# kenziyuliu/ChineseCheckersAgent

Hardware: NVIDIA B200
Metric: env_steps_per_sec (higher is better)
Workload: dtype u64

## Files before the change

chinesecheckersagent_b200/csrc/ccx_device.cuh:

```cuda
#pragma once
#include <cstdint>
#include <cuda_runtime.h>

typedef unsigned long long u64;
typedef unsigned int u32;

#define CCX_HD __host__ __device__ __forceinline__
#ifdef __CUDA_ARCH__
#define ccx_popc(x) __popc(x)
#define ccx_popcll(x) __popcll(x)
#define ccx_umulhi(a, b) __umulhi((a), (b))
#define ccx_clz(x) __clz(x)
#define ccx_clzll(x) __clzll((long long)(x))
#define ccx_ffs(x) __ffs(x)
#else
#define ccx_popc(x) __builtin_popcount(x)
#define ccx_popcll(x) __builtin_popcountll(x)
#define ccx_umulhi(a, b) ((u32)(((u64)(u32)(a) * (u64)(u32)(b)) >> 32))
#define ccx_clz(x) ((x) ? __builtin_clz(x) : 32)
#define ccx_clzll(x) ((x) ? __builtin_clzll(x) : 64)
#define ccx_ffs(x) __builtin_ffs(x)
#endif

#define CCX_VALID 0x007F7F7F7F7F7F7FULL
// ... 330 lines not shown

CCX_HD void apply_move(Game &g, int id, int from, int to)
{
    g.occ_me ^= (1ULL << from) | (1ULL << to);
    g.cells_me = (g.cells_me & ~(0xFFULL << (8 * id))) | ((u64)to << (8 * id));
    u64 meta = g.meta;
    u64 ply = ((meta >> 32) + 1) & 0xFFFF;
    g.meta = (meta & 0xFFFF000000000000ULL) ^ (1ULL << 48) | (ply << 32) | ((meta & 0xFFFF) << 16) |
             (u64)from | ((u64)to << 8);
    u64 t;
    t = g.occ_me; g.occ_me = g.occ_op; g.occ_op = t;
    t = g.cells_me; g.cells_me = g.cells_op; g.cells_op = t;
}

CCX_HD void push_hist(u64 &lo, u64 &hi, int to)
{
    hi = (hi << 8) | (lo >> 56);
    lo = (lo << 8) | (u64)to;
}

CCX_HD int level_of(int cell) { return (cell >> 3) - (cell & 7) + 6; }

CCX_HD int winner_of(const Game &g)
{
    bool p2 = (g.meta >> 48) & 1;
    return check_win(p2 ? g.occ_op : g.occ_me, p2 ? g.occ_me : g.occ_op);
}

CCX_HD void reset_start(Game &g)
{
    g.occ_me = CCX_START_OCC1; g.occ_op = CCX_START_OCC2;
    g.cells_me = CCX_START_CELLS1; g.cells_op = CCX_START_CELLS2;
    g.meta = CCX_START_META;
}

CCX_HD int pick_random(const Game &g, const u64 (&dest)[6], u32 nonempty, u32 r0, u32 r1, int &from, int &to)
{
    int j = (int)ccx_umulhi(r0, nonempty);
    int id = 0, rank = 0; u64 m = 0;
#pragma unroll
    for (int k = 0; k < 6; k++) {
        bool ne = dest[k] != 0;
        if (ne && rank == j) { id = k; m = dest[k]; }
        rank += ne;
    }
    to = select64(m, ccx_umulhi(r1, (u32)ccx_popcll(m)));
    from = (int)((g.cells_me >> (8 * id)) & 0xFF);
    return id;
}

struct TriTables {
    const uint8_t *sT; const u64 *sNB, *sCI, *sO, *sOT, *sOD;
    const u32 *sSel;
};

CCX_HD void tri_build(u64 cells_a, u64 cells_b, const u64 *__restrict__ sOT, const u64 *__restrict__ sOD, u64 &occT, u64 &occD)
{
    occT = 0; occD = 0;
#pragma unroll
    for (int k = 0; k < 6; k++) {
        int a = (int)((cells_a >> (8 * k)) & 0x3F), b = (int)((cells_b >> (8 * k)) & 0x3F);
        occT |= sOT[a] | sOT[b];
        occD |= sOD[a] | sOD[b];
    }
}

CCX_HD void movegen_tri(u64 occ_all, u64 occT_all, u64 occD_all, u64 cells, u64 (&dest)[6], const TriTables &T)
{
#pragma unroll
    for (int k = 0; k < 6; k++) dest[k] = 0;
    int id = 0, cell = (int)(cells & 0x3F);
    u64 o = T.sO[cell], occ = occ_all & ~o, occT = occT_all & ~T.sOT[cell], occD = occD_all & ~T.sOD[cell];
    u64 todo = o, reach = 0;
    for (;;) {
        int c = 63 - ccx_clzll(todo);
        todo ^= T.sO[c];
        u64 nw = expand_cell_tri(c, occ, occT, occD, T.sT, T.sCI) & ~(reach | o);
        reach |= nw;
        todo |= nw;
        if (todo == 0) {
            u64 d = (T.sNB[cell] & ~occ) | reach;
#pragma unroll
            for (int k = 0; k < 6; k++) if (id == k) dest[k] = d;
            if (++id == 6) break;
            cell = (int)((cells >> (8 * id)) & 0x3F);
            o = T.sO[cell]; occ = occ_all & ~o; occT = occT_all & ~T.sOT[cell]; occD = occD_all & ~T.sOD[cell];
            todo = o; reach = 0;
        }
    }
}

struct JumpFill {
    u64 o, occ, occT, occD, todo, reach;
};

CCX_HD JumpFill fill_start(int cell, u64 occ_all, u64 occT_all, u64 occD_all, const TriTables &T)
{
    JumpFill f;
    f.o = 1ULL << cell;
    f.occ = occ_all & ~f.o; f.occT = occT_all & ~T.sOT[cell]; f.occD = occD_all & ~T.sOD[cell];
    f.todo = f.o; f.reach = 0;
    return f;
}

CCX_HD void fill_step(JumpFill &f, const TriTables &T)
{
    const int c = 63 - ccx_clzll(f.todo);
    f.todo ^= 1ULL << c;
    const u64 nw = expand_cell_tri(c, f.occ, f.occT, f.occD, T.sT, T.sCI) & ~(f.reach | f.o);
    f.reach |= nw;
    f.todo |= nw;
}

CCX_HD u32 walk_movable(u64 occ_me, u64 occ_all, u64 cells_me)
{
    const u64 w = occ_me & neighbours(~occ_all & CCX_VALID);
    u32 b = 0;
#pragma unroll
    for (int k = 0; k < 6; k++) b |= (u32)((w >> ((cells_me >> (8 * k)) & 0x3F)) & 1) << k;
    return b;
}

CCX_HD int pick_first_start(const Game &g, u64 occT_all, u64 occD_all, u32 r0, const TriTables &T, int &from, JumpFill &f)
{
    const u64 occ_all = g.occ_me | g.occ_op;
    u32 movable = walk_movable(g.occ_me, occ_all, g.cells_me);
    u32 nowalk = ~movable & 0x3Fu;
    while (nowalk) {
        const int k = ccx_ffs(nowalk) - 1;
        nowalk &= nowalk - 1;
// ... 44 lines not shown
    k -= up ? c : 0u;
    const u32 c1 = ccx_popc(w & 0xFFu), c2 = ccx_popc(w & 0xFFFFu), c3 = ccx_popc(w & 0xFFFFFFu);
    const bool p1 = k >= c1, p2 = k >= c2, p3 = k >= c3;
    const u32 below = p2 ? (p3 ? c3 : c2) : (p1 ? c1 : 0u);
    const u32 sh = p2 ? (p3 ? 24u : 16u) : (p1 ? 8u : 0u);
    const u32 v = (w >> sh) & 0xFFu, r = k - below;
    const u32 pos = r < (u32)ccx_popc(v & 0x7Fu) ? sel7_rank(sSel, v & 0x7Fu, r) : 7u;
    return (int)((up ? 32u : 0u) + sh + pos);
}

CCX_HD u32 walk_movable_step(u64 occ_me, u64 occ_all, u64 cells_me)
{
    const u64 w = (occ_me & neighbours(~occ_all & CCX_VALID)) << 8;
    const u32 slo = (u32)cells_me + 0x05060708u, shi = (u32)(cells_me >> 32) + 0x0304u;
    u32 b = 0;
#pragma unroll
    for (u32 k = 0; k < 6; k++) b |= (u32)(w >> ccx_byte_of(slo, shi, 0x8880u | k)) & (1u << k);
    return b;
}

#define CCX_DBASE_LO 0x78503018u
#define CCX_DBASE_HI 0x305078A8u
struct CarryCell { u32 rsel, csel, dsel, lp8, sh; };
CCX_HD CarryCell carry_cell(int c)
{
    const int r = c >> 3, col = c & 7, k = col - r;
    const u32 x = (u32)k + 0x8894u;
    const u32 base8 = ccx_byte_of(CCX_DBASE_LO, CCX_DBASE_HI, 0x8894u - (u32)k);
    CarryCell q;
    q.rsel = 0x8880u | (u32)r;
    q.csel = 0x8880u | (u32)col;
    q.dsel = x & ((x - 1u) | 7u);
    q.lp8 = base8 + 8u * (u32)(r < col ? r : col);
    q.sh = (u32)(k > -8 * k ? k : -8 * k);
    return q;
}

CCX_HD u64 expand_cell_carry(int c, u64 occ, u64 occT, u64 occD, const uint8_t *__restrict__ T3)
{
    CarryCell q = carry_cell(c);
    const int r8 = c & 0x38;
    const u32 row7 = ccx_byte_of((u32)occ, (u32)(occ >> 32), q.rsel);
    u64 L = (u64)T3[CCX_JT3_ROW + row7 * 64 + c] << r8;
    const u32 col7 = ccx_byte_of((u32)occT, (u32)(occT >> 32), q.csel);
    L |= *reinterpret_cast<const u64 *>(T3 + CCX_JT3_COL + col7 * 64 + r8) << (c & 7);
    const u32 dia7 = ccx_byte_of((u32)occD, (u32)(occD >> 32), q.dsel);
#ifdef __CUDA_ARCH__
    asm("" : "+r"(q.lp8));
#endif
    L |= *reinterpret_cast<const u64 *>(T3 + CCX_JT3_DIA + dia7 * (CCX_JT3_NLP * 8) + q.lp8) << q.sh;
    return L;
}

CCX_HD void fill_step_carry(JumpFill &f, const uint8_t *__restrict__ T3)
{
    const int h = ccx_flo((u32)(f.todo >> 32)) | 32, l = ccx_flo((u32)f.todo);
    const int c = h > l ? h : l;
    f.todo ^= 1ULL << c;
    const u64 nw = expand_cell_carry(c, f.occ, f.occT, f.occD, T3) & ~(f.reach | f.o);
    f.reach |= nw;
    f.todo |= nw;
}

CCX_HD JumpFill carry_fill_start(int from, u64 occ_all, u64 occT_all, u64 occD_all, const TriTables &T)
{
    JumpFill f;
    f.o = 1ULL << from;
    f.occ = occ_all & ~f.o; f.occT = occT_all & ~T.sOT[from]; f.occD = occD_all & ~T.sOD[from];
    f.todo = expand_cell_carry(from, occ_all, occT_all, occD_all, T.sT);
    f.reach = (T.sNB[from] & ~occ_all) | f.todo;
    return f;
}

CCX_HD int carry_ply_start(const Game &g, u64 occT_all, u64 occD_all, u32 r0, const TriTables &T, int &from, JumpFill &f)
{
    const u64 occ_all = g.occ_me | g.occ_op;
    u32 movable = walk_movable_step(g.occ_me, occ_all, g.cells_me);
    u32 nowalk = ~movable & 0x3Fu;
    while (nowalk) {
        const int k = ccx_ffs(nowalk) - 1;
        nowalk &= nowalk - 1;
        if (expand_cell_carry((int)((g.cells_me >> (8 * k)) & 0x3F), occ_all, occT_all, occD_all, T.sT)) movable |= 1u << k;
    }
    if (!movable) return -1;
    const int id = (int)sel7_rank(T.sSel, movable, ccx_umulhi(r0, (u32)ccx_popc(movable)));
    from = (int)ccx_byte_of((u32)g.cells_me, (u32)(g.cells_me >> 32), 0x8880u | (u32)id);
    f = carry_fill_start(from, occ_all, occT_all, occD_all, T);
    return id;
}

CCX_HD int carry_ply_to(const JumpFill &f, u32 r1, const TriTables &T)
{
    return select64_step(f.reach, ccx_umulhi(r1, (u32)ccx_popcll(f.reach)), T.sSel);
}

CCX_HD u64 diag_mask(int l)
{
    const u64 D0 = 0x0040201008040201ULL;
    int k = 6 - l;
    if (k >= 0) return (D0 << k) & ((1ULL << (8 * (7 - k))) - 1ULL) & CCX_VALID;
    return (D0 << (8 * (-k))) & CCX_VALID;
}

CCX_HD int greedy_candidates(const Game &g, const u64 (&dest)[6], u64 (&cand)[6])
{
    bool p2 = (g.meta >> 48) & 1;
    int dist[6], start[6];
    int max_dist = -100;
#pragma unroll
    for (int k = 0; k < 6; k++) {
        u32 levels = 0;
#pragma unroll
        for (int l = 0; l < 13; l++) {
            const u64 dm = diag_mask(l);
            levels |= (dest[k] & dm) ? (1u << l) : 0u;
        }
        start[k] = level_of((int)((g.cells_me >> (8 * k)) & 0xFF));
        int best_end = p2 ? (31 - ccx_clz(levels)) : (ccx_ffs(levels) - 1);
        dist[k] = levels ? (p2 ? best_end - start[k] : start[k] - best_end) : -100;
        max_dist = dist[k] > max_dist ? dist[k] : max_dist;
    }
    int s_star = p2 ? 100 : -100;
#pragma unroll
    for (int k = 0; k < 6; k++)
        if (dist[k] == max_dist) s_star = p2 ? (start[k] < s_star ? start[k] : s_star) : (start[k] > s_star ? start[k] : s_star);
    int total = 0;
    if (max_dist == -100) {
#pragma unroll
        for (int k = 0; k < 6; k++) cand[k] = 0;
        return 0;
    }
    u64 end_mask = diag_mask(p2 ? s_star + max_dist : s_star - max_dist);
#pragma unroll
    for (int k = 0; k < 6; k++) {
        cand[k] = (dist[k] == max_dist && start[k] == s_star) ? (dest[k] & end_mask) : 0;
        total += ccx_popcll(cand[k]);
    }
    return total;
}

// ... 34 lines not shown
```

chinesecheckersagent_b200/csrc/ccx_env.cu:

```cuda
#include <cuda_bf16.h>
#include <new>
#include <cstdlib>
#include "ccx_device.cuh"
#include "ccx_internal.h"

#ifndef CCX_GREEDY_DEFAULT_VARIANT
#define CCX_GREEDY_DEFAULT_VARIANT 1
#endif
#define ENV_THREADS 64
#define ENC_THREADS 128


__device__ __forceinline__ Game load_game(const u64 *__restrict__ st, int64_t n, int64_t i)
{
    u64 occ1 = st[0 * n + i], occ2 = st[1 * n + i], c1 = st[2 * n + i], c2 = st[3 * n + i];
    Game g;
    g.meta = st[4 * n + i];
    bool p2 = (g.meta >> 48) & 1;
    g.occ_me = p2 ? occ2 : occ1; g.occ_op = p2 ? occ1 : occ2;
    g.cells_me = p2 ? c2 : c1;   g.cells_op = p2 ? c1 : c2;
    return g;
}

__device__ __forceinline__ void store_game(u64 *__restrict__ st, int64_t n, int64_t i, const Game &g)
// ... 71 lines not shown
    if (i >= n) return;
    Game g = load_game(st, n, i);
    int f = from[i], t = to[i];
    int id = 0;
#pragma unroll
    for (int k = 5; k >= 0; k--) if (((g.cells_me >> (8 * k)) & 0xFF) == (u64)f) id = k;
    apply_move(g, id, f, t);
    store_game(st, n, i, g);
    u64 lo = st[5 * n + i], hi = st[6 * n + i];
    push_hist(lo, hi, t);
    st[5 * n + i] = lo; st[6 * n + i] = hi;
    winner[i] = (uint8_t)winner_of(g);
}

__global__ void __launch_bounds__(ENV_THREADS)
k_info(const u64 *__restrict__ st, int64_t n, int16_t *__restrict__ out)
{
    int64_t i = (int64_t)blockIdx.x * blockDim.x + threadIdx.x;
    if (i >= n) return;
    u64 occ1 = st[0 * n + i], occ2 = st[1 * n + i], c1 = st[2 * n + i], c2 = st[3 * n + i];
    int d1 = 70, d2 = -14;
#pragma unroll
    for (int k = 0; k < 6; k++) {
        d1 -= level_of((int)((c1 >> (8 * k)) & 0xFF)) + 1;
        d2 += level_of((int)((c2 >> (8 * k)) & 0xFF)) + 1;
    }
    out[i * 5 + 0] = (int16_t)check_win(occ1, occ2);
    out[i * 5 + 1] = (int16_t)__popcll(occ1 & CCX_TARGET_P1);
    out[i * 5 + 2] = (int16_t)__popcll(occ2 & CCX_TARGET_P2);
    out[i * 5 + 3] = (int16_t)d1;
    out[i * 5 + 4] = (int16_t)d2;
}


#define CCX_TRI_SMEM_BYTES (CCX_JT3_BYTES + 5 * 64 * 8)
template <int TPB, bool SEL = false>
__device__ __forceinline__ TriTables tri_tables_load(uint8_t *sAll, const uint8_t *__restrict__ jt3)
{
    u64 *sNB = reinterpret_cast<u64 *>(sAll + CCX_JT3_BYTES), *sCI = sNB + 64, *sO = sNB + 128, *sOT = sNB + 192, *sOD = sNB + 256;
    u32 *sSel = SEL ? reinterpret_cast<u32 *>(sAll + CCX_TRI_SMEM_BYTES) : nullptr;
    for (int q = threadIdx.x; q < CCX_JT3_BYTES / 16; q += TPB) reinterpret_cast<uint4 *>(sAll)[q] = reinterpret_cast<const uint4 *>(jt3)[q];
    for (int q = threadIdx.x; q < 64; q += TPB) {
        const bool on = (CCX_VALID >> q) & 1;
        sNB[q] = on ? (neighbours(1ULL << q) & CCX_VALID) : 0ULL;
        sCI[q] = on ? tri_cell_info(q) : 0ULL;
        sO[q] = 1ULL << q;
        sOT[q] = on ? 1ULL << tri_tbit(q) : 0ULL;
        sOD[q] = on ? 1ULL << tri_dbit(q) : 0ULL;
    }
    if (SEL)
        for (int q = threadIdx.x; q < 128; q += TPB) sSel[q] = sel7_entry((u32)q);
    __syncthreads();
    TriTables t = {sAll, sNB, sCI, sO, sOT, sOD, sSel};
    return t;
}

template <bool TRACE, int TPB, int MINB>
__global__ void __launch_bounds__(TPB, MINB, 1)
k_step_random_pick(u64 *__restrict__ st, int64_t n, int64_t gid0, u32 k0, u32 k1, u32 step0, int plies,
                   u64 *__restrict__ wins, u64 *__restrict__ trace, int64_t trace_games, const uint8_t *__restrict__ jt3)
{
    __shared__ __align__(16) uint8_t sAll[CCX_JT3_BYTES + 5 * 64 * 8];
    const TriTables T = tri_tables_load<TPB>(sAll, jt3);
    const int64_t i = (int64_t)blockIdx.x * TPB + threadIdx.x;
    if (i >= n) return;
    Game g = load_game(st, n, i);
    const u64 gid = (u64)(gid0 + i);
    u32 w1 = 0, w2 = 0;
    u64 occT_all, occD_all;
    tri_build(g.cells_me, g.cells_op, T.sOT, T.sOD, occT_all, occD_all);
    for (int t = 0; t < plies; t++) {
        u64 *row = nullptr;
        if (TRACE && i < trace_games) {
            row = trace + ((int64_t)t * trace_games + i) * CCX_TRACE_WORDS;
            u64 dest[6];
            movegen_tri(g.occ_me | g.occ_op, occT_all, occD_all, g.cells_me, dest, T);
            bool p2 = (g.meta >> 48) & 1;
            row[0] = p2 ? g.occ_op : g.occ_me; row[1] = p2 ? g.occ_me : g.occ_op;
            row[2] = p2 ? g.cells_op : g.cells_me; row[3] = p2 ? g.cells_me : g.cells_op;
            row[4] = g.meta & 0x00FFFFFFFFFFFFFFULL;
#pragma unroll
            for (int q = 0; q < 6; q++) row[5 + q] = dest[q];
            row[11] = 0xFFULL | (0xFFULL << 8) | (0xFFULL << 24);
        }
        Philox4 rnd = philox4x32_10(k0, k1, step0 + (u32)t, 0u, (u32)gid, (u32)(gid >> 32));
        int from, to;
        const int pid = pick_random_first(g, occT_all, occD_all, rnd.x, rnd.y, T, from, to);
        if (pid < 0) continue;
        apply_move(g, pid, from, to);
        occT_all ^= T.sOT[from] | T.sOT[to];
        occD_all ^= T.sOD[from] | T.sOD[to];
        const int win = winner_of(g);
        if (TRACE && row) row[11] = (u64)from | ((u64)to << 8) | ((u64)win << 16) | ((u64)pid << 24);
        if (win) { w1 += win == 1; w2 += win == 2; reset_start(g); tri_build(g.cells_me, g.cells_op, T.sOT, T.sOD, occT_all, occD_all); }
    }
    store_game(st, n, i, g);
    if (w1) atomicAdd(&wins[0], (u64)w1);
    if (w2) atomicAdd(&wins[1], (u64)w2);
}

template <bool TRACE, int TPB, int MINB, int K>
__global__ void __launch_bounds__(TPB, MINB, 1)
k_step_random_carry(u64 *__restrict__ st, int64_t n, int64_t gid0, u32 k0, u32 k1, u32 step0, int plies,
                    u64 *__restrict__ wins, u64 *__restrict__ trace, int64_t trace_games, const uint8_t *__restrict__ jt3)
{
    __shared__ __align__(16) uint8_t sAll[CCX_TRI_SMEM_BYTES + CCX_SEL7_BYTES];
    const TriTables T = tri_tables_load<TPB, true>(sAll, jt3);
    const int64_t i = (int64_t)blockIdx.x * TPB + threadIdx.x;
    if (i >= n) return;
    Game g = load_game(st, n, i);
    const u64 gid = (u64)(gid0 + i);
    u32 w1 = 0, w2 = 0;
    JumpFill f = {0, 0, 0, 0, 0, 0};
    tri_build(g.cells_me, g.cells_op, T.sOT, T.sOD, f.occT, f.occD);
    int t = 0, id = -1, from = 0;
    Philox4 rnd = philox4x32_10(k0, k1, step0, 0u, (u32)gid, (u32)(gid >> 32));
    u32 r1 = 0;
    for (;;) {
        if (!f.todo) {
            u64 occT_all = f.occT, occD_all = f.occD;
            if (id >= 0) {
                rnd = philox4x32_10(k0, k1, step0 + (u32)t + 1u, 0u, (u32)gid, (u32)(gid >> 32));
                const int to = carry_ply_to(f, r1, T);
                apply_move(g, id, from, to);
                occT_all |= T.sOT[to];
                occD_all |= T.sOD[to];
#ifdef __CUDA_ARCH__
                asm volatile("" ::"r"(rnd.x), "r"(rnd.y));
#endif
                const int win = winner_of(g);
                if (TRACE && i < trace_games)
                    trace[((int64_t)t * trace_games + i) * CCX_TRACE_WORDS + 11] = (u64)from | ((u64)to << 8) | ((u64)win << 16) | ((u64)id << 24);
                if (win) { w1 += win == 1; w2 += win == 2; reset_start(g); tri_build(g.cells_me, g.cells_op, T.sOT, T.sOD, occT_all, occD_all); }
                t++;
                id = -1;
            }
            for (; t < plies; t++) {
                if (TRACE && i < trace_games) {
                    u64 *row = trace + ((int64_t)t * trace_games + i) * CCX_TRACE_WORDS;
                    u64 dest[6];
                    movegen_tri(g.occ_me | g.occ_op, occT_all, occD_all, g.cells_me, dest, T);
                    bool p2 = (g.meta >> 48) & 1;
                    row[0] = p2 ? g.occ_op : g.occ_me; row[1] = p2 ? g.occ_me : g.occ_op;
                    row[2] = p2 ? g.cells_op : g.cells_me; row[3] = p2 ? g.cells_me : g.cells_op;
                    row[4] = g.meta & 0x00FFFFFFFFFFFFFFULL;
#pragma unroll
                    for (int q = 0; q < 6; q++) row[5 + q] = dest[q];
                    row[11] = 0xFFULL | (0xFFULL << 8) | (0xFFULL << 24);
                }
                r1 = rnd.y;
                id = carry_ply_start(g, occT_all, occD_all, rnd.x, T, from, f);
                if (id >= 0) break;
                rnd = philox4x32_10(k0, k1, step0 + (u32)t + 1u, 0u, (u32)gid, (u32)(gid >> 32));
            }
            if (id < 0) break;
        }
#pragma unroll
        for (int k = 0; k < K; k++) { if (!f.todo) break; fill_step_carry(f, T.sT); }
    }
    store_game(st, n, i, g);
    if (w1) atomicAdd(&wins[0], (u64)w1);
    if (w2) atomicAdd(&wins[1], (u64)w2);
}

template <bool TRACE, int TPB, int MINB, bool PRE>
__global__ void __launch_bounds__(TPB, MINB, 1)
k_step_random_wq(u64 *__restrict__ st, int64_t n, int64_t gid0, u32 k0, u32 k1, u32 step0, int plies,
                 u64 *__restrict__ wins, u64 *__restrict__ trace, int64_t trace_games, const uint8_t *__restrict__ jt3)
{
    extern __shared__ __align__(16) u64 sDyn[];
    __shared__ __align__(16) uint8_t sAll[CCX_JT3_BYTES + 5 * 64 * 8];
    const uint8_t *sT = sAll;
    u64 *sNB = reinterpret_cast<u64 *>(sAll + CCX_JT3_BYTES);
    u64 *sCI = reinterpret_cast<u64 *>(sAll + CCX_JT3_BYTES + 512);
    u64 *sO = reinterpret_cast<u64 *>(sAll + CCX_JT3_BYTES + 1024);
    u64 *sOT = reinterpret_cast<u64 *>(sAll + CCX_JT3_BYTES + 1536);
    u64 *sOD = reinterpret_cast<u64 *>(sAll + CCX_JT3_BYTES + 2048);
    const int tid = threadIdx.x, lane = tid & 31, warp = tid >> 5;
    for (int q = tid; q < CCX_JT3_BYTES / 16; q += TPB) reinterpret_cast<uint4 *>(sAll)[q] = reinterpret_cast<const uint4 *>(jt3)[q];
    for (int q = tid; q < 64; q += TPB) {
        const bool on = (CCX_VALID >> q) & 1;
        sNB[q] = on ? (neighbours(1ULL << q) & CCX_VALID) : 0ULL;
        sCI[q] = on ? tri_cell_info(q) : 0ULL;
        sO[q] = 1ULL << q;
        sOT[q] = on ? 1ULL << tri_tbit(q) : 0ULL;
        sOD[q] = on ? 1ULL << tri_dbit(q) : 0ULL;
    }
    __syncthreads();
    constexpr int WARP_WORDS = PRE ? (6 + 4 * 6) * 32 : 10 * 32;
    u64 *sD = sDyn + warp * WARP_WORDS;
    u64 *sG = sD + 6 * 32;
    const int64_t i = (int64_t)blockIdx.x * TPB + tid;
    const bool act = i < n;
    Game g = load_game(st, n, act ? i : 0);
    if (!act) reset_start(g);
    const u64 gid = (u64)(gid0 + i);
    u32 w1 = 0, w2 = 0;
    u64 occT_all, occD_all;
    tri_build(g.cells_me, g.cells_op, sOT, sOD, occT_all, occD_all);
    const unsigned lt_mask = (1u << lane) - 1u;
    for (int t = 0; t < plies; t++) {
        const u64 occ_all = g.occ_me | g.occ_op;
        if (PRE) {
#pragma unroll
            for (int q = 0; q < 6; q++) {
                const int cell = (int)((g.cells_me >> (8 * q)) & 0x3F);
                const u64 oq = 1ULL << cell;
                sG[0 * 192 + q * 32 + lane] = oq;
                sG[1 * 192 + q * 32 + lane] = occ_all & ~oq;
                sG[2 * 192 + q * 32 + lane] = occT_all & ~sOT[cell];
                sG[3 * 192 + q * 32 + lane] = occD_all & ~sOD[cell];
// ... 26 lines not shown
                        todo = o; reach = 0; state = 1;
                    } else state = 2;
                }
                if (working == 0) break;
            }
            if (state == 1) {
                const int c = 63 - __clzll((long long)todo);
                todo ^= PRE ? 1ULL << c : sO[c];
                const u64 nw = expand_cell_tri(c, occ, occT, occD, sT, sCI) & ~(reach | o);
                reach |= nw;
                todo |= nw;
                if (todo == 0) { sD[PRE ? gi : k * 32 + gi] = reach; state = 0; }
            }
        }
        __syncwarp();
        u64 dest[6];
#pragma unroll
        for (int q = 0; q < 6; q++) dest[q] = sD[q * 32 + lane] | (sNB[(g.cells_me >> (8 * q)) & 0x3F] & ~occ_all);
        u32 nonempty = 0;
#pragma unroll
        for (int q = 0; q < 6; q++) nonempty += dest[q] != 0;
        u64 *row = nullptr;
        if (TRACE && i < trace_games) {
            row = trace + ((int64_t)t * trace_games + i) * CCX_TRACE_WORDS;
            bool p2 = (g.meta >> 48) & 1;
            row[0] = p2 ? g.occ_op : g.occ_me; row[1] = p2 ? g.occ_me : g.occ_op;
            row[2] = p2 ? g.cells_op : g.cells_me; row[3] = p2 ? g.cells_me : g.cells_op;
            row[4] = g.meta & 0x00FFFFFFFFFFFFFFULL;
#pragma unroll
            for (int q = 0; q < 6; q++) row[5 + q] = dest[q];
            row[11] = 0xFFULL | (0xFFULL << 8) | (0xFFULL << 24);
        }
        if (nonempty) {
            Philox4 rnd = philox4x32_10(k0, k1, step0 + (u32)t, 0u, (u32)gid, (u32)(gid >> 32));
            int from, to;
            int pid = pick_random(g, dest, nonempty, rnd.x, rnd.y, from, to);
            apply_move(g, pid, from, to);
            occT_all ^= sOT[from] | sOT[to];
            occD_all ^= sOD[from] | sOD[to];
            int win = winner_of(g);
            if (TRACE && row) row[11] = (u64)from | ((u64)to << 8) | ((u64)win << 16) | ((u64)pid << 24);
            if (win) { w1 += win == 1; w2 += win == 2; reset_start(g); tri_build(g.cells_me, g.cells_op, sOT, sOD, occT_all, occD_all); }
        }
        __syncwarp();
    }
    if (!act) return;
    store_game(st, n, i, g);
    if (w1) atomicAdd(&wins[0], (u64)w1);
    if (w2) atomicAdd(&wins[1], (u64)w2);
}


__global__ void k_build_jump_table3(uint8_t *T3) { build_jump_table3(T3, blockIdx.x * blockDim.x + threadIdx.x, gridDim.x * blockDim.x); }


__global__ void __launch_bounds__(ENV_THREADS)
k_greedy_candidates(const u64 *__restrict__ st, int64_t n, u64 *__restrict__ masks, const uint8_t *__restrict__ jt)
{
    LOAD_JUMP_TABLE(sT, jt)
    int64_t i = (int64_t)blockIdx.x * blockDim.x + threadIdx.x;
    if (i >= n) return;
    Game g = load_game(st, n, i);
    u64 dest[6], cand[6];
    movegen_rays(g.occ_me | g.occ_op, g.cells_me, dest, sT);
    greedy_candidates(g, dest, cand);
#pragma unroll
    for (int k = 0; k < 6; k++) masks[k * n + i] = cand[k];
}

__global__ void __launch_bounds__(ENV_THREADS)
k_play_greedy(u64 *__restrict__ st, int64_t n, int64_t gid0, u32 k0, u32 k1, int max_plies,
              u64 *__restrict__ counters, const uint8_t *__restrict__ jt)
{
    LOAD_JUMP_TABLE(sT, jt)
    int64_t i = (int64_t)blockIdx.x * blockDim.x + threadIdx.x;
    u32 played = 0, w1 = 0, w2 = 0, rep = 0;
    if (i < n) {
        Game g = load_game(st, n, i);
        u64 lo = st[5 * n + i], hi = st[6 * n + i];
        u64 gid = (u64)(gid0 + i);
        int status = (int)(g.meta >> 56);
        for (int t = 0; status == CCX_ST_RUNNING && t < max_plies; t++) {
            u64 dest[6], cand[6];
            movegen_rays(g.occ_me | g.occ_op, g.cells_me, dest, sT);
            int total = greedy_candidates(g, dest, cand);
            if (total == 0) { status = CCX_ST_NO_MOVES; break; }
            u32 ply = (u32)((g.meta >> 32) & 0xFFFF);
            Philox4 r = philox4x32_10(k0, k1, ply, 1u, (u32)gid, (u32)(gid >> 32));
            int from, to;
            int id = pick_candidate(g, cand, total, r.x, from, to);
            apply_move(g, id, from, to);
            push_hist(lo, hi, to);
            played++;
            int win = winner_of(g);
            if (win) { status = win; w1 += win == 1; w2 += win == 2; break; }
            if (((g.meta >> 32) & 0xFFFF) >= 16 && repetition_stop(lo, hi)) { status = CCX_ST_REPETITION; rep++; }
        }
        g.meta = (g.meta & 0x00FFFFFFFFFFFFFFULL) | ((u64)status << 56);
        store_game(st, n, i, g);
        st[5 * n + i] = lo; st[6 * n + i] = hi;
    }
    if (counters) {
        for (int off = 16; off; off >>= 1) {
            played += __shfl_down_sync(0xFFFFFFFFu, played, off);
            w1 += __shfl_down_sync(0xFFFFFFFFu, w1, off);
            w2 += __shfl_down_sync(0xFFFFFFFFu, w2, off);
// ... 102 lines not shown
        if (p2)
            for (int c = 0; c < 49; c++) t[c * 7 + 6] = enc_val<T>(1);
    }
    __syncthreads();
    char *dst = reinterpret_cast<char *>(out) + g0 * 343 * (int64_t)sizeof(T);
    int bytes = games * 343 * (int)sizeof(T);
    int nvec = bytes / 16;
    uint4 *dst4 = reinterpret_cast<uint4 *>(dst);
    for (int v = threadIdx.x; v < nvec; v += blockDim.x) dst4[v] = smem_u4[v];
    const char *src = reinterpret_cast<const char *>(smem_u4);
    for (int b = nvec * 16 + threadIdx.x; b < bytes; b += blockDim.x) dst[b] = src[b];
}


static inline unsigned blocks_for(int64_t n, int per) { return (unsigned)((n + per - 1) / per); }

extern "C" {

int ccx_abi_version(void) { return CCX_ABI_VERSION; }

const char *ccx_strerror(int code)
{
    switch (code) {
    case CCX_OK: return "ok";
    case CCX_ERR_ARG: return "invalid argument";
    case CCX_ERR_CUDA: return "CUDA error (see ccx_last_cuda_error)";
    case CCX_ERR_NOMEM: return "out of device memory";
    case CCX_ERR_STATE: return "invalid handle state";
    case CCX_ERR_UNSUPPORTED: return "unsupported";
    case CCX_ERR_OVERFLOW: return "node pool overflow";
    default: return "unknown error";
    }
}

const char *ccx_last_cuda_error(const ccx_handle *h) { return h ? h->cuda_err : ""; }

int ccx_create(int device_ordinal, ccx_handle **out)
{
    if (!out) return CCX_ERR_ARG;
    *out = nullptr;
    int count = 0;
    cudaError_t e = cudaGetDeviceCount(&count);
    if (e != cudaSuccess || device_ordinal < 0 || device_ordinal >= count) return e != cudaSuccess ? CCX_ERR_CUDA : CCX_ERR_ARG;
    ccx_handle *h = new (std::nothrow) ccx_handle();
    if (!h) return CCX_ERR_NOMEM;
    h->device = device_ordinal;
    if (cudaSetDevice(device_ordinal) != cudaSuccess) { delete h; return CCX_ERR_CUDA; }
    cudaDeviceProp prop;
    if (cudaGetDeviceProperties(&prop, device_ordinal) == cudaSuccess) h->num_sms = prop.multiProcessorCount;
    if (cudaMalloc(&h->jump_table, CCX_JT_BYTES) != cudaSuccess) { delete h; return CCX_ERR_NOMEM; }
    k_build_jump_table<<<7, 128>>>(h->jump_table);
    if (cudaMalloc(&h->jump_table3, CCX_JT3_BYTES) != cudaSuccess) { cudaFree(h->jump_table); delete h; return CCX_ERR_NOMEM; }
    k_build_jump_table3<<<28, 128>>>(h->jump_table3);
    if (cudaDeviceSynchronize() != cudaSuccess) { cudaFree(h->jump_table); cudaFree(h->jump_table3); delete h; return CCX_ERR_CUDA; }
    *out = h;
    return CCX_OK;
}

int ccx_destroy(ccx_handle *h)
{
    if (!h) return CCX_OK;
    cudaSetDevice(h->device);
    ccx_net_free(h);
    ccx_net_tc_free(h);
    ccx_net_acc_free(h);
    ccx_trees_free(h);
    ccx_scratch *s[] = {&h->d_state, &h->d_aux0, &h->d_aux1, &h->d_aux2};
    for (auto *p : s) if (p->ptr) cudaFree(p->ptr);
    if (h->jump_table) cudaFree(h->jump_table);
    if (h->jump_table3) cudaFree(h->jump_table3);
    if (h->ev_fork) cudaEventDestroy(h->ev_fork);
    if (h->ev_join) cudaEventDestroy(h->ev_join);
    if (h->stream2) cudaStreamDestroy(h->stream2);
    delete h;
    return CCX_OK;
}

int ccx_set_stream(ccx_handle *h, void *cuda_stream)
{
    if (!h) return CCX_ERR_ARG;
    h->stream = (cudaStream_t)cuda_stream;
    return CCX_OK;
}

int ccx_synchronize(ccx_handle *h)
{
    if (!h) return CCX_ERR_ARG;
    CCX_CUDA(h, cudaStreamSynchronize(h->stream));
    return CCX_OK;
}

int64_t ccx_launch_count(const ccx_handle *h) { return h ? h->launches : 0; }
int64_t ccx_graph_replays(const ccx_handle *h) { return h ? h->graph_replays : 0; }

int ccx_reset(ccx_handle *h, int64_t n, uint64_t *state, int mode, uint64_t seed, int64_t game_id0)
{
    if (!h || n < 0 || (n && !state) || (mode != CCX_RESET_START && mode != CCX_RESET_RANDOMISED)) return CCX_ERR_ARG;
    if (n == 0) return CCX_OK;
    k_reset<<<blocks_for(n, ENV_THREADS), ENV_THREADS, 0, h->stream>>>((u64 *)state, n, mode, (u32)seed, (u32)(seed >> 32), game_id0);
    CCX_LAUNCHED(h);
    return CCX_OK;
}

int ccx_movegen(ccx_handle *h, int64_t n, const uint64_t *state, uint64_t *dest_masks)
{
    if (!h || n < 0 || (n && (!state || !dest_masks))) return CCX_ERR_ARG;
    if (n == 0) return CCX_OK;
    k_movegen<<<blocks_for(n, ENV_THREADS), ENV_THREADS, 0, h->stream>>>((const u64 *)state, n, (u64 *)dest_masks, h->jump_table);
    CCX_LAUNCHED(h);
    return CCX_OK;
}

int ccx_apply(ccx_handle *h, int64_t n, uint64_t *state, const uint8_t *from, const uint8_t *to, uint8_t *winner)
{
    if (!h || n < 0 || (n && (!state || !from || !to || !winner))) return CCX_ERR_ARG;
    if (n == 0) return CCX_OK;
    k_apply<<<blocks_for(n, ENV_THREADS), ENV_THREADS, 0, h->stream>>>((u64 *)state, n, from, to, winner);
    CCX_LAUNCHED(h);
    return CCX_OK;
}

int ccx_info(ccx_handle *h, int64_t n, const uint64_t *state, int16_t *out)
{
    if (!h || n < 0 || (n && (!state || !out))) return CCX_ERR_ARG;
    if (n == 0) return CCX_OK;
    k_info<<<blocks_for(n, ENV_THREADS), ENV_THREADS, 0, h->stream>>>((const u64 *)state, n, out);
    CCX_LAUNCHED(h);
    return CCX_OK;
}

int ccx_step_random(ccx_handle *h, int64_t n, uint64_t *state, int64_t game_id0, uint64_t seed, uint32_t step0,
                    int32_t plies, uint64_t *wins, uint64_t *trace, int64_t trace_games)
{
    if (!h || n < 0 || plies < 0 || (n && (!state || !wins)) || (trace_games > 0 && !trace)) return CCX_ERR_ARG;
    if (n == 0 || plies == 0) return CCX_OK;
    const char *ve = getenv("CCX_STEP_VARIANT");
    const int variant = ve ? atoi(ve) : 11;
    if (variant < 9 || variant > 11) return CCX_ERR_ARG;
    const u32 s0 = (u32)seed, s1 = (u32)(seed >> 32);
    const bool tr = trace && trace_games > 0;
    u64 *tp = tr ? (u64 *)trace : nullptr;
    const int64_t tg = tr ? trace_games : 0;
    const bool one_wave = n <= (int64_t)h->num_sms * 448;
    if (variant == 11) {
#define CCX_CARRY_LAUNCH(TR, MINB, K)                                                                                            \
        k_step_random_carry<TR, 448, MINB, K><<<blocks_for(n, 448), 448, 0, h->stream>>>((u64 *)state, n, game_id0, s0, s1, step0, \
                                                                                         plies, (u64 *)wins, tp, tg, h->jump_table3)
        if (one_wave) { if (tr) CCX_CARRY_LAUNCH(true, 1, 5); else CCX_CARRY_LAUNCH(false, 1, 5); }
        else { if (tr) CCX_CARRY_LAUNCH(true, 2, 4); else CCX_CARRY_LAUNCH(false, 2, 4); }
#undef CCX_CARRY_LAUNCH
    } else if (variant == 10) {
#define CCX_PICK_LAUNCH(TR, MINB)                                                                                                \
        k_step_random_pick<TR, 448, MINB><<<blocks_for(n, 448), 448, 0, h->stream>>>((u64 *)state, n, game_id0, s0, s1, step0, plies, \
                                                                                     (u64 *)wins, tp, tg, h->jump_table3)
        if (one_wave) { if (tr) CCX_PICK_LAUNCH(true, 1); else CCX_PICK_LAUNCH(false, 1); }
        else { if (tr) CCX_PICK_LAUNCH(true, 2); else CCX_PICK_LAUNCH(false, 2); }
#undef CCX_PICK_LAUNCH
    } else {
#define CCX_WQ_LAUNCH(TR, TPB, MINB, PRE)                                                                                        \
        do {                                                                                                                      \
            static bool attr_set = false;                                                                                         \
            constexpr int DYN = (TPB / 32) * ((PRE) ? 30 : 10) * 32 * 8;                                                           \
            if (!attr_set) {                                                                                                      \
                CCX_CUDA(h, cudaFuncSetAttribute(k_step_random_wq<TR, TPB, MINB, PRE>, cudaFuncAttributeMaxDynamicSharedMemorySize, DYN)); \
                attr_set = true;                                                                                                  \
            }                                                                                                                     \
            k_step_random_wq<TR, TPB, MINB, PRE><<<blocks_for(n, TPB), TPB, DYN, h->stream>>>(                                     \
                (u64 *)state, n, game_id0, s0, s1, step0, plies, (u64 *)wins, tp, tg, h->jump_table3);                              \
        } while (0)
        if (one_wave) { if (tr) CCX_WQ_LAUNCH(true, 448, 1, true); else CCX_WQ_LAUNCH(false, 448, 1, true); }
        else { if (tr) CCX_WQ_LAUNCH(true, 448, 2, false); else CCX_WQ_LAUNCH(false, 448, 2, false); }
#undef CCX_WQ_LAUNCH
    }
    CCX_LAUNCHED(h);
    return CCX_OK;
}

int ccx_greedy_candidates(ccx_handle *h, int64_t n, const uint64_t *state, uint64_t *cand_masks)
{
    if (!h || n < 0 || (n && (!state || !cand_masks))) return CCX_ERR_ARG;
    if (n == 0) return CCX_OK;
    k_greedy_candidates<<<blocks_for(n, ENV_THREADS), ENV_THREADS, 0, h->stream>>>((const u64 *)state, n, (u64 *)cand_masks, h->jump_table);
    CCX_LAUNCHED(h);
    return CCX_OK;
}

int ccx_play_greedy(ccx_handle *h, int64_t n, uint64_t *state, int64_t game_id0, uint64_t seed, int32_t max_plies,
                    uint64_t *counters)
{
    if (!h || n < 0 || max_plies < 0 || (n && !state)) return CCX_ERR_ARG;
    if (n == 0 || max_plies == 0) return CCX_OK;
    const char *ve = getenv("CCX_GREEDY_VARIANT");
    const int variant = ve ? atoi(ve) : CCX_GREEDY_DEFAULT_VARIANT;
    if (variant == 1)
        k_play_greedy_tri<448, 2><<<blocks_for(n, 448), 448, 0, h->stream>>>((u64 *)state, n, game_id0, (u32)seed, (u32)(seed >> 32), max_plies, (u64 *)counters, h->jump_table3);
    else if (variant == 2)
        k_play_greedy_tri<224, 4><<<blocks_for(n, 224), 224, 0, h->stream>>>((u64 *)state, n, game_id0, (u32)seed, (u32)(seed >> 32), max_plies, (u64 *)counters, h->jump_table3);
    else if (variant == 3)
        k_play_greedy_tri<128, 4><<<blocks_for(n, 128), 128, 0, h->stream>>>((u64 *)state, n, game_id0, (u32)seed, (u32)(seed >> 32), max_plies, (u64 *)counters, h->jump_table3);
    else
// ... 132 lines not shown
```

chinesecheckersagent_b200/csrc/ccx_internal.h:

```cpp
#pragma once
#include <cuda_runtime.h>
#include <cstdint>
#include <cstdio>
#include <cstring>
#include "../../include/ccx.h"

struct ccx_scratch {
    void *ptr = nullptr;
    size_t bytes = 0;
};

struct ccx_net;
struct ccx_trees;
struct ccx_net_tc;
struct ccx_net_acc;

struct ccx_handle {
    int device = 0;
    int num_sms = 148;
    cudaStream_t stream = nullptr;
    int64_t launches = 0;
    char cuda_err[256] = {0};
    ccx_scratch d_state, d_aux0, d_aux1, d_aux2;
    ccx_net *net = nullptr;
    ccx_trees *trees = nullptr;
    ccx_net_tc *net_tc = nullptr;
    ccx_net_acc *net_acc = nullptr;
    uint8_t *jump_table = nullptr;
    uint8_t *jump_table3 = nullptr;
    const int64_t *slot_ids = nullptr;
    int tie_mode = 0;
    uint64_t tie_seed = 0;
    int64_t tie_uid0 = 0;
    int net_mode = 0;
    int acc_ctx = -1;
    cudaStream_t stream2 = nullptr;
    cudaEvent_t ev_fork = nullptr, ev_join = nullptr;
    uint64_t epoch = 0;
    uint64_t pool_gen = 1;
    uint64_t search_gen = 0;
    int64_t search_n = 0;
    void *round_graph = nullptr;
    void *leaf_pool = nullptr;
    void *reuse_pool = nullptr;
    cudaStream_t cap_stream = nullptr;
    int graph_off = 0;
    int64_t graph_replays = 0;
};

static inline int ccx_fail(ccx_handle *h, cudaError_t e)
{
    if (h) snprintf(h->cuda_err, sizeof(h->cuda_err), "%s: %s", cudaGetErrorName(e), cudaGetErrorString(e));
    return e == cudaErrorMemoryAllocation ? CCX_ERR_NOMEM : CCX_ERR_CUDA;
}

#define CCX_CUDA(h, call)                                   \
    do {                                                    \
        cudaError_t e__ = (call);                           \
        if (e__ != cudaSuccess) return ccx_fail((h), e__);  \
    } while (0)

#define CCX_LAUNCHED(h)                                     \
    do {                                                    \
        (h)->launches++;                                    \
        cudaError_t e__ = cudaGetLastError();               \
        if (e__ != cudaSuccess) return ccx_fail((h), e__);  \
    } while (0)

static inline int ccx_reserve(ccx_handle *h, ccx_scratch &s, size_t bytes)
{
    if (s.bytes >= bytes) return CCX_OK;
    if (s.ptr) { CCX_CUDA(h, cudaFree(s.ptr)); s.ptr = nullptr; s.bytes = 0; }
    size_t want = bytes + bytes / 4;
    CCX_CUDA(h, cudaMalloc(&s.ptr, want));
    s.bytes = want;
    return CCX_OK;
}

int ccx_net_scratch(ccx_handle *h, int64_t n, uint8_t **planes, float **logits, float **value);
int ccx_net_forward_active(ccx_handle *h, int64_t n, const uint8_t *planes, float *logits, float *value);
int ccx_net_forward_tc_on(ccx_handle *h, cudaStream_t stream, int64_t cap, int64_t row0, int64_t n, const uint8_t *planes, float *logits,
                          float *value);
// ... 14 lines not shown
```

Baseline: 31.86 billion.

## Use pre-shifted wide u64 jump tables in shared memory for one-wave carry kernel

Adds a precomputed 192KB table of pre-shifted u64 jump masks (row, column, diagonal) built from the byte table at init. The one-wave carry random-rollout kernel loads it into dynamic shared memory, so each cell expansion becomes three shared loads ORed together with no per-lookup shifts or offset math. The trade-off is a much larger shared-memory footprint per block, a longer table load at kernel start, and reliance on inline PTX shared loads.

```diff
diff --git a/chinesecheckersagent_b200/csrc/ccx_device.cuh b/chinesecheckersagent_b200/csrc/ccx_device.cuh
--- a/chinesecheckersagent_b200/csrc/ccx_device.cuh
+++ b/chinesecheckersagent_b200/csrc/ccx_device.cuh
@@ -406,6 +406,7 @@
 struct TriTables {
     const uint8_t *sT; const u64 *sNB, *sCI, *sO, *sOT, *sOD;
     const u32 *sSel;
+    const u64 *sW;
 };
 
 CCX_HD void tri_build(u64 cells_a, u64 cells_b, const u64 *__restrict__ sOT, const u64 *__restrict__ sOD, u64 &occT, u64 &occD)
@@ -419,6 +420,8 @@
     }
 }
 
+CCX_HD u64 expand_cell_carry(int c, u64 occ, u64 occT, u64 occD, const u64 *__restrict__ W);
+template <bool WIDE = false>
 CCX_HD void movegen_tri(u64 occ_all, u64 occT_all, u64 occD_all, u64 cells, u64 (&dest)[6], const TriTables &T)
 {
 #pragma unroll
@@ -429,7 +432,7 @@
     for (;;) {
         int c = 63 - ccx_clzll(todo);
         todo ^= T.sO[c];
-        u64 nw = expand_cell_tri(c, occ, occT, occD, T.sT, T.sCI) & ~(reach | o);
+        u64 nw = (WIDE ? expand_cell_carry(c, occ, occT, occD, T.sW) : expand_cell_tri(c, occ, occT, occD, T.sT, T.sCI)) & ~(reach | o);
         reach |= nw;
         todo |= nw;
         if (todo == 0) {
@@ -580,26 +583,70 @@
     return L;
 }
 
-CCX_HD void fill_step_carry(JumpFill &f, const uint8_t *__restrict__ T3)
+#define CCX_JTW_ROW 0
+#define CCX_JTW_COL (128 * 64)
+#define CCX_JTW_DIA (2 * 128 * 64)
+#define CCX_JTW_BYTES (3 * 128 * 64 * 8)
+CCX_HD void build_jump_table_wide(u64 *W, const uint8_t *T3, int first, int step)
+{
+    for (int e = first; e < 128 * 64; e += step) {
+        const int o7 = e / 64, c = e % 64, r = c >> 3, col = c & 7, k = col - r;
+        const bool on = (CCX_VALID >> c) & 1, dia = on && k >= -4 && k <= 4;
+        const u64 ci = tri_cell_info(c);
+        W[CCX_JTW_ROW + e] = on ? (u64)T3[CCX_JT3_ROW + o7 * 64 + c] << (c & 0x38) : 0;
+        W[CCX_JTW_COL + e] = on ? *reinterpret_cast<const u64 *>(T3 + CCX_JT3_COL + o7 * 64 + 8 * r) << col : 0;
+        W[CCX_JTW_DIA + e] = dia ? *reinterpret_cast<const u64 *>(T3 + CCX_JT3_DIA + o7 * (CCX_JT3_NLP * 8) + ((u32)ci >> 24))
+                                       << ((ci >> 16) & 0xFF) : 0;
+    }
+}
+
+CCX_HD u64 expand_cell_carry(int c, u64 occ, u64 occT, u64 occD, const u64 *__restrict__ W)
+{
+    const CarryCell q = carry_cell(c);
+    const u32 row7 = ccx_byte_of((u32)occ, (u32)(occ >> 32), q.rsel);
+    const u32 col7 = ccx_byte_of((u32)occT, (u32)(occT >> 32), q.csel);
+    const u32 dia7 = ccx_byte_of((u32)occD, (u32)(occD >> 32), q.dsel);
+#ifdef __CUDA_ARCH__
+    const u32 wc = (u32)__cvta_generic_to_shared(W) + 8u * (u32)c;
+    u64 a, b, d;
+    asm("ld.shared.u64 %0, [%1];" : "=l"(a) : "r"(wc + row7 * 512u));
+    asm("ld.shared.u64 %0, [%1+65536];" : "=l"(b) : "r"(wc + col7 * 512u));
+    asm("ld.shared.u64 %0, [%1+131072];" : "=l"(d) : "r"(wc + dia7 * 512u));
+    return a | b | d;
+#else
+    return W[CCX_JTW_ROW + row7 * 64 + c] | W[CCX_JTW_COL + col7 * 64 + c] | W[CCX_JTW_DIA + dia7 * 64 + c];
+#endif
+}
+
+template <bool WIDE>
+CCX_HD auto carry_tables(const TriTables &T)
+{
+    if constexpr (WIDE) return T.sW; else return T.sT;
+}
+
+template <class TAB>
+CCX_HD void fill_step_carry(JumpFill &f, const TAB *__restrict__ tab)
 {
     const int h = ccx_flo((u32)(f.todo >> 32)) | 32, l = ccx_flo((u32)f.todo);
     const int c = h > l ? h : l;
     f.todo ^= 1ULL << c;
-    const u64 nw = expand_cell_carry(c, f.occ, f.occT, f.occD, T3) & ~(f.reach | f.o);
+    const u64 nw = expand_cell_carry(c, f.occ, f.occT, f.occD, tab) & ~(f.reach | f.o);
     f.reach |= nw;
     f.todo |= nw;
 }
 
+template <bool WIDE = false>
 CCX_HD JumpFill carry_fill_start(int from, u64 occ_all, u64 occT_all, u64 occD_all, const TriTables &T)
 {
     JumpFill f;
     f.o = 1ULL << from;
     f.occ = occ_all & ~f.o; f.occT = occT_all & ~T.sOT[from]; f.occD = occD_all & ~T.sOD[from];
-    f.todo = expand_cell_carry(from, occ_all, occT_all, occD_all, T.sT);
+    f.todo = expand_cell_carry(from, occ_all, occT_all, occD_all, carry_tables<WIDE>(T));
     f.reach = (T.sNB[from] & ~occ_all) | f.todo;
     return f;
 }
 
+template <bool WIDE = false>
 CCX_HD int carry_ply_start(const Game &g, u64 occT_all, u64 occD_all, u32 r0, const TriTables &T, int &from, JumpFill &f)
 {
     const u64 occ_all = g.occ_me | g.occ_op;
@@ -608,12 +655,13 @@
     while (nowalk) {
         const int k = ccx_ffs(nowalk) - 1;
         nowalk &= nowalk - 1;
-        if (expand_cell_carry((int)((g.cells_me >> (8 * k)) & 0x3F), occ_all, occT_all, occD_all, T.sT)) movable |= 1u << k;
+        if (expand_cell_carry((int)((g.cells_me >> (8 * k)) & 0x3F), occ_all, occT_all, occD_all, carry_tables<WIDE>(T)))
+            movable |= 1u << k;
     }
     if (!movable) return -1;
     const int id = (int)sel7_rank(T.sSel, movable, ccx_umulhi(r0, (u32)ccx_popc(movable)));
     from = (int)ccx_byte_of((u32)g.cells_me, (u32)(g.cells_me >> 32), 0x8880u | (u32)id);
-    f = carry_fill_start(from, occ_all, occT_all, occD_all, T);
+    f = carry_fill_start<WIDE>(from, occ_all, occT_all, occD_all, T);
     return id;
 }
 
diff --git a/chinesecheckersagent_b200/csrc/ccx_env.cu b/chinesecheckersagent_b200/csrc/ccx_env.cu
--- a/chinesecheckersagent_b200/csrc/ccx_env.cu
+++ b/chinesecheckersagent_b200/csrc/ccx_env.cu
@@ -147,6 +147,35 @@
         for (int q = threadIdx.x; q < 128; q += TPB) sSel[q] = sel7_entry((u32)q);
     __syncthreads();
     TriTables t = {sAll, sNB, sCI, sO, sOT, sOD, sSel};
+    return t;
+}
+
+#define CCX_WIDE_SMEM_BYTES (CCX_JTW_BYTES + 4 * 64 * 8 + CCX_SEL7_BYTES)
+template <int TPB>
+__device__ __forceinline__ TriTables wide_tables_load(uint8_t *s, const u64 *__restrict__ jtw)
+{
+    u64 *sW = reinterpret_cast<u64 *>(s), *sNB = sW + 3 * 128 * 64, *sO = sNB + 64, *sOT = sNB + 128, *sOD = sNB + 192;
+    u32 *sSel = reinterpret_cast<u32 *>(sNB + 256);
+    constexpr int N = CCX_JTW_BYTES / 16, U = 4;
+    const uint4 *src = reinterpret_cast<const uint4 *>(jtw);
+    uint4 *dst = reinterpret_cast<uint4 *>(s);
+    for (int q = threadIdx.x; q < N; q += U * TPB) {
+        uint4 v[U];
+#pragma unroll
+        for (int u = 0; u < U; u++) if (q + u * TPB < N) v[u] = src[q + u * TPB];
+#pragma unroll
+        for (int u = 0; u < U; u++) if (q + u * TPB < N) dst[q + u * TPB] = v[u];
+    }
+    for (int q = threadIdx.x; q < 64; q += TPB) {
+        const bool on = (CCX_VALID >> q) & 1;
+        sNB[q] = on ? (neighbours(1ULL << q) & CCX_VALID) : 0ULL;
+        sO[q] = 1ULL << q;
+        sOT[q] = on ? 1ULL << tri_tbit(q) : 0ULL;
+        sOD[q] = on ? 1ULL << tri_dbit(q) : 0ULL;
+    }
+    for (int q = threadIdx.x; q < 128; q += TPB) sSel[q] = sel7_entry((u32)q);
+    __syncthreads();
+    TriTables t = {nullptr, sNB, nullptr, sO, sOT, sOD, sSel, sW};
     return t;
 }
 
@@ -197,10 +226,13 @@
 template <bool TRACE, int TPB, int MINB, int K>
 __global__ void __launch_bounds__(TPB, MINB, 1)
 k_step_random_carry(u64 *__restrict__ st, int64_t n, int64_t gid0, u32 k0, u32 k1, u32 step0, int plies,
-                    u64 *__restrict__ wins, u64 *__restrict__ trace, int64_t trace_games, const uint8_t *__restrict__ jt3)
-{
-    __shared__ __align__(16) uint8_t sAll[CCX_TRI_SMEM_BYTES + CCX_SEL7_BYTES];
-    const TriTables T = tri_tables_load<TPB, true>(sAll, jt3);
+                    u64 *__restrict__ wins, u64 *__restrict__ trace, int64_t trace_games, const uint8_t *__restrict__ jt3,
+                    const u64 *__restrict__ jtw)
+{
+    constexpr bool WIDE = MINB == 1;
+    extern __shared__ __align__(16) u64 sDyn[];
+    __shared__ __align__(16) uint8_t sAll[WIDE ? 16 : CCX_TRI_SMEM_BYTES + CCX_SEL7_BYTES];
+    const TriTables T = WIDE ? wide_tables_load<TPB>(reinterpret_cast<uint8_t *>(sDyn), jtw) : tri_tables_load<TPB, true>(sAll, jt3);
     const int64_t i = (int64_t)blockIdx.x * TPB + threadIdx.x;
     if (i >= n) return;
     Game g = load_game(st, n, i);
@@ -234,7 +266,7 @@
                 if (TRACE && i < trace_games) {
                     u64 *row = trace + ((int64_t)t * trace_games + i) * CCX_TRACE_WORDS;
                     u64 dest[6];
-                    movegen_tri(g.occ_me | g.occ_op, occT_all, occD_all, g.cells_me, dest, T);
+                    movegen_tri<WIDE>(g.occ_me | g.occ_op, occT_all, occD_all, g.cells_me, dest, T);
                     bool p2 = (g.meta >> 48) & 1;
                     row[0] = p2 ? g.occ_op : g.occ_me; row[1] = p2 ? g.occ_me : g.occ_op;
                     row[2] = p2 ? g.cells_op : g.cells_me; row[3] = p2 ? g.cells_me : g.cells_op;
@@ -244,14 +276,14 @@
                     row[11] = 0xFFULL | (0xFFULL << 8) | (0xFFULL << 24);
                 }
                 r1 = rnd.y;
-                id = carry_ply_start(g, occT_all, occD_all, rnd.x, T, from, f);
+                id = carry_ply_start<WIDE>(g, occT_all, occD_all, rnd.x, T, from, f);
                 if (id >= 0) break;
                 rnd = philox4x32_10(k0, k1, step0 + (u32)t + 1u, 0u, (u32)gid, (u32)(gid >> 32));
             }
             if (id < 0) break;
         }
 #pragma unroll
-        for (int k = 0; k < K; k++) { if (!f.todo) break; fill_step_carry(f, T.sT); }
+        for (int k = 0; k < K; k++) { if (!f.todo) break; fill_step_carry(f, carry_tables<WIDE>(T)); }
     }
     store_game(st, n, i, g);
     if (w1) atomicAdd(&wins[0], (u64)w1);
@@ -384,6 +416,7 @@
 
 
 __global__ void k_build_jump_table3(uint8_t *T3) { build_jump_table3(T3, blockIdx.x * blockDim.x + threadIdx.x, gridDim.x * blockDim.x); }
+__global__ void k_build_jump_table_wide(u64 *W, const uint8_t *T3) { build_jump_table_wide(W, T3, blockIdx.x * blockDim.x + threadIdx.x, gridDim.x * blockDim.x); }
 
 
 __global__ void __launch_bounds__(ENV_THREADS)
@@ -592,7 +625,11 @@
     k_build_jump_table<<<7, 128>>>(h->jump_table);
     if (cudaMalloc(&h->jump_table3, CCX_JT3_BYTES) != cudaSuccess) { cudaFree(h->jump_table); delete h; return CCX_ERR_NOMEM; }
     k_build_jump_table3<<<28, 128>>>(h->jump_table3);
-    if (cudaDeviceSynchronize() != cudaSuccess) { cudaFree(h->jump_table); cudaFree(h->jump_table3); delete h; return CCX_ERR_CUDA; }
+    if (cudaMalloc(&h->jump_table_wide, CCX_JTW_BYTES) != cudaSuccess) { cudaFree(h->jump_table); cudaFree(h->jump_table3); delete h; return CCX_ERR_NOMEM; }
+    k_build_jump_table_wide<<<64, 128>>>((u64 *)h->jump_table_wide, h->jump_table3);
+    if (cudaDeviceSynchronize() != cudaSuccess) {
+        cudaFree(h->jump_table); cudaFree(h->jump_table3); cudaFree(h->jump_table_wide); delete h; return CCX_ERR_CUDA;
+    }
     *out = h;
     return CCX_OK;
 }
@@ -609,6 +646,7 @@
     for (auto *p : s) if (p->ptr) cudaFree(p->ptr);
     if (h->jump_table) cudaFree(h->jump_table);
     if (h->jump_table3) cudaFree(h->jump_table3);
+    if (h->jump_table_wide) cudaFree(h->jump_table_wide);
     if (h->ev_fork) cudaEventDestroy(h->ev_fork);
     if (h->ev_join) cudaEventDestroy(h->ev_join);
     if (h->stream2) cudaStreamDestroy(h->stream2);
@@ -683,9 +721,14 @@
     const int64_t tg = tr ? trace_games : 0;
     const bool one_wave = n <= (int64_t)h->num_sms * 448;
     if (variant == 11) {
+        if (one_wave && !h->carry_wide_smem) {
+            CCX_CUDA(h, cudaFuncSetAttribute(k_step_random_carry<false, 448, 1, 5>, cudaFuncAttributeMaxDynamicSharedMemorySize, CCX_WIDE_SMEM_BYTES));
+            CCX_CUDA(h, cudaFuncSetAttribute(k_step_random_carry<true, 448, 1, 5>, cudaFuncAttributeMaxDynamicSharedMemorySize, CCX_WIDE_SMEM_BYTES));
+            h->carry_wide_smem = true;
+        }
 #define CCX_CARRY_LAUNCH(TR, MINB, K)                                                                                            \
-        k_step_random_carry<TR, 448, MINB, K><<<blocks_for(n, 448), 448, 0, h->stream>>>((u64 *)state, n, game_id0, s0, s1, step0, \
-                                                                                         plies, (u64 *)wins, tp, tg, h->jump_table3)
+        k_step_random_carry<TR, 448, MINB, K><<<blocks_for(n, 448), 448, (MINB) == 1 ? CCX_WIDE_SMEM_BYTES : 0, h->stream>>>(     \
+            (u64 *)state, n, game_id0, s0, s1, step0, plies, (u64 *)wins, tp, tg, h->jump_table3, (const u64 *)h->jump_table_wide)
         if (one_wave) { if (tr) CCX_CARRY_LAUNCH(true, 1, 5); else CCX_CARRY_LAUNCH(false, 1, 5); }
         else { if (tr) CCX_CARRY_LAUNCH(true, 2, 4); else CCX_CARRY_LAUNCH(false, 2, 4); }
 #undef CCX_CARRY_LAUNCH
diff --git a/chinesecheckersagent_b200/csrc/ccx_internal.h b/chinesecheckersagent_b200/csrc/ccx_internal.h
--- a/chinesecheckersagent_b200/csrc/ccx_internal.h
+++ b/chinesecheckersagent_b200/csrc/ccx_internal.h
@@ -28,6 +28,8 @@
     ccx_net_acc *net_acc = nullptr;
     uint8_t *jump_table = nullptr;
     uint8_t *jump_table3 = nullptr;
+    uint8_t *jump_table_wide = nullptr;
+    bool carry_wide_smem = false;
     const int64_t *slot_ids = nullptr;
     int tie_mode = 0;
     uint64_t tie_seed = 0;
```

Result: faster. 37.27 billion, median of 6 (+17.0%).
